# flashlight/wav2letter

Measured on NVIDIA H100. Metric: frames_per_sec, higher is better.
Workload: dtype f32

## Files before the change

### include/w2l_b200.h

```cpp
#ifndef W2L_B200_H_
#define W2L_B200_H_

#include <stddef.h>
#include <stdint.h>

#ifdef __cplusplus
extern "C" {
#endif

#define W2L_API __attribute__((visibility("default")))

enum {
  W2L_OK = 0,
  W2L_ERR_INVALID_ARGUMENT = 1,
  W2L_ERR_WORKSPACE = 2,
  W2L_ERR_CUDA = 3,
  W2L_ERR_UNSUPPORTED = 4
};

enum {
  W2L_SCALE_NONE = 0,
  W2L_SCALE_INPUT_SZ = 1,
  W2L_SCALE_INPUT_SZ_SQRT = 2,
  W2L_SCALE_TARGET_SZ = 3,
// ... 84 lines not shown
W2L_API int w2l_seq2seq_beam_finish(void* stream, int B, int K, int maxlen, int steps, int pad, const void* ws, size_t ws_bytes, int32_t* tokens,
                                    int32_t* lengths, float* scores, int32_t* counts);

W2L_API int w2l_soft_label_loss(void* stream, long long rows, int N, const float* student, const float* teacher, float scale, float* loss_out,
                                float* d_student, float* ws);
W2L_API int w2l_ema_update(void* stream, long long n, float* ema, const float* params, double decay);

W2L_API int w2l_gemm_tf32_view(void* stream, int a_mn_major, int b_mn_major, int M, int N, int K, const float* A, int lda,
                               const float* B, int ldb, float* C, int ldc, const float* bias, int act, int accumulate);
enum { W2L_GEMM_TF32 = 0, W2L_GEMM_F32X3 = 1, W2L_GEMM_BF16 = 2, W2L_GEMM_F32X3_SPLIT_B = 3, W2L_GEMM_FP16 = 4 };
enum { W2L_PRECISION_TF32 = 0, W2L_PRECISION_F32 = 1, W2L_PRECISION_BF16 = 2, W2L_PRECISION_FP16 = 3 };
W2L_API int w2l_set_precision(int precision);
W2L_API int w2l_get_precision(void);
W2L_API int w2l_gemm(void* stream, int kind, int a_mn_major, int b_mn_major, int M, int N, int K, const void* A, int lda,
                     const void* B, int ldb, void* C, int ldc, int c_bf16, const float* bias, int act, int accumulate,
                     const void* aux, int ld_aux, int aux_bf16, int aux_mode, float aux_scale, float dropout_p,
                     unsigned long long seed, int allow_overlap);
W2L_API int w2l_cast_bf16(void* stream, long long n, const float* x, void* y);
W2L_API int w2l_cast_bf16_rows(void* stream, long long rows, int cols, int ld_in, int cols_padded, const float* x, void* y);
W2L_API int w2l_cast_fp16(void* stream, long long n, const float* x, void* y);
W2L_API int w2l_cast_fp16_rows(void* stream, long long rows, int cols, int ld_in, int cols_padded, const float* x, void* y);
W2L_API int w2l_split_tf32(void* stream, int transpose, int rows, int cols, int ld, int cols_padded, const float* x, float* planes);
W2L_API int w2l_gemm_set_tile(int bn);
W2L_API int w2l_gemm_set_variant(int variant);
W2L_API int w2l_gemm_tf32(void* stream, int a_mn_major, int b_mn_major, int M, int N, int K, const float* A, int lda,
                          const float* B, int ldb, float* C, int ldc, const float* bias, int act);

W2L_API int w2l_gemm_tf32_ex(void* stream, int a_mn_major, int b_mn_major, int M, int N, int K, const float* A, int lda,
                             const float* B, int ldb, float* C, int ldc, const float* bias, int act, int accumulate,
                             const float* aux, int ld_aux, int aux_mode, float aux_scale, float dropout_p,
                             unsigned long long seed);

W2L_API size_t w2l_conv_time_workspace_size(int B, int Tout, int Cin, int Cout, int K);
W2L_API int w2l_conv_time_fwd(void* stream, int B, int T, int Tout, int W, int Cin, int Cout, int K, int stride,
                              int pad_left, const float* x, const float* wt, const float* bias, const float* add, float* y,
                              int act, float dropout_p, unsigned long long seed, void* ws, size_t ws_bytes);
W2L_API int w2l_conv_time_dgrad(void* stream, int B, int T, int Tout, int W, int Cin, int Cout, int K, int stride,
                                int pad_left, const float* dy, const float* wt, const float* add, float* dx, void* ws,
                                size_t ws_bytes);
W2L_API int w2l_conv_time_wgrad(void* stream, int B, int T, int Tout, int W, int Cin, int Cout, int K, int stride,
                                int pad_left, const float* x, const float* dy, float* dwt, float* dbias, void* ws,
                                size_t ws_bytes);

W2L_API int w2l_weightnorm_fwd(void* stream, int rows, int len, const float* v, const float* g, float* w, float* inv_norm);
W2L_API int w2l_weightnorm_bwd(void* stream, int rows, int len, const float* v, const float* g, const float* inv_norm,
                               const float* dw, float* dv, float* dg);
// ... 143 lines not shown
```

### wav2letter_b200/capi.py

```python
from __future__ import annotations

import ctypes
import os

import torch

_HERE = os.path.dirname(os.path.abspath(__file__))
LIB_PATH = os.path.join(_HERE, "libw2l_b200.so")

SCALE_MODES = {"none": 0, "input_sz": 1, "input_sz_sqrt": 2, "target_sz": 3, "target_sz_sqrt": 4}
TERM_FCC, TERM_FAC, TERM_ASG = 1, 2, 3

EXPORTS = [
    "w2l_version", "w2l_last_error", "w2l_launch_count", "w2l_reset_launch_count", "w2l_set_profile_events", "w2l_set_profile_event_list", "w2l_profile_events_used", "w2l_trace_begin", "w2l_trace_end", "w2l_trace_list",
    "w2l_asg_workspace_size", "w2l_asg_forward_backward",
    "w2l_asg64_workspace_size", "w2l_asg64_forward_backward",
    "w2l_fcc_viterbi_workspace_size", "w2l_fcc_viterbi",
    "w2l_fcc_viterbi64_workspace_size", "w2l_fcc_viterbi64",
    "w2l_fac_viterbi_workspace_size", "w2l_fac_viterbi",
    "w2l_ctc_workspace_size", "w2l_ctc_forward_backward", "w2l_argmax_path", "w2l_linseg_target",
    "w2l_ctc_viterbi_workspace_size", "w2l_ctc_viterbi_target",
    "w2l_set_precision", "w2l_get_precision", "w2l_gemm", "w2l_cast_bf16", "w2l_cast_bf16_rows", "w2l_cast_fp16", "w2l_cast_fp16_rows", "w2l_split_tf32", "w2l_sgd_step_ex", "w2l_finite_guard",
    "w2l_mask_bands", "w2l_trainer_set_precision", "w2l_trainer_set_grad_stream", "w2l_trainer_set_grad_stream_delay", "w2l_delay", "w2l_trainer_status", "w2l_trainer_save", "w2l_trainer_load", "w2l_trainer_export_streaming",
    "w2l_trainer_set_schedule", "w2l_trainer_set_position", "w2l_trainer_position", "w2l_trainer_set_lr", "w2l_trainer_lr",
    "w2l_trainer_set_amp", "w2l_trainer_amp_state",
    "w2l_text_create", "w2l_text_destroy", "w2l_text_num_classes", "w2l_text_encode", "w2l_text_prediction2ltr", "w2l_text_target2ltr",
    "w2l_text_ltr2wrd", "w2l_text_align_words", "w2l_edit_distance",
    "w2l_gemm_set_variant", "w2l_gemm_set_tile", "w2l_gemm_tf32", "w2l_gemm_tf32_ex", "w2l_gemm_tf32_view", "w2l_conv_time_workspace_size", "w2l_conv_time_fwd", "w2l_conv_time_dgrad",
    "w2l_conv_time_wgrad", "w2l_layernorm_fwd", "w2l_layernorm_rows_fwd", "w2l_layernorm_bwd", "w2l_colsum_accumulate", "w2l_sq_norm_accumulate",
    "w2l_sgd_step", "w2l_weightnorm_fwd", "w2l_weightnorm_bwd", "w2l_conv1d_arrange", "w2l_conv1d_arrange_ex", "w2l_conv1d_unarrange_grad",
    "w2l_glu_fwd", "w2l_glu_bwd", "w2l_prelu_fwd", "w2l_prelu_bwd", "w2l_transpose_input", "w2l_axpy", "w2l_fill", "w2l_act_fwd", "w2l_mask_mul",
    "w2l_trainer_create", "w2l_trainer_destroy", "w2l_trainer_step", "w2l_trainer_forward", "w2l_trainer_num_params",
    "w2l_trainer_param_layout", "w2l_trainer_get_flat", "w2l_trainer_set_flat", "w2l_trainer_sync_parameters",
    "w2l_trainer_describe", "w2l_nccl_unique_id", "w2l_init_distributed", "w2l_trainer_align", "w2l_trainer_time_stride",
    "w2l_mfsc_num_frames", "w2l_mfsc_workspace_size", "w2l_mfsc",
    "w2l_stream_create", "w2l_stream_destroy", "w2l_stream_state_bytes", "w2l_stream_max_frames_out", "w2l_stream_start",
    "w2l_stream_run", "w2l_stream_plan",
    "w2l_mfsc_stream_create", "w2l_mfsc_stream_destroy", "w2l_mfsc_stream_state_bytes", "w2l_mfsc_stream_max_frames_out",
    "w2l_mfsc_stream_start", "w2l_mfsc_stream_run",
    "w2l_seq2seq_check", "w2l_seq2seq_embed_fwd", "w2l_seq2seq_embed_bwd", "w2l_seq2seq_gru_stash_floats", "w2l_seq2seq_gru_fwd",
    "w2l_seq2seq_gru_bwd", "w2l_seq2seq_attn_fwd", "w2l_seq2seq_attn_bwd", "w2l_seq2seq_loss", "w2l_seq2seq_scale_rows",
    "w2l_seq2seq_decode_init", "w2l_seq2seq_decode_step",
    "w2l_seq2seq_beam_workspace_size", "w2l_seq2seq_beam_init", "w2l_seq2seq_beam_step", "w2l_seq2seq_beam_finish",
    "w2l_trainer_create_seq2seq", "w2l_trainer_output_width", "w2l_trainer_seq2seq_config", "w2l_trainer_clear_window",
    "w2l_trainer_seq2seq_seed", "w2l_trainer_decode", "w2l_trainer_beam_search",
    "w2l_seq2seq_sizes", "w2l_seq2seq_attn_fwd_sized", "w2l_seq2seq_attn_bwd_sized", "w2l_trainer_step_sized", "w2l_trainer_decode_sized",
    "w2l_trainer_beam_search_sized",
    "w2l_soft_label_loss", "w2l_ema_update", "w2l_trainer_set_ema", "w2l_trainer_ema", "w2l_trainer_forward_teacher",
    "w2l_trainer_viterbi_path", "w2l_trainer_step_soft",
]

# ... 465 lines not shown
    _check(lib.w2l_cast_fp16_rows(_stream(), x.shape[0], x.shape[1], x.stride(0), cols_padded, _ptr(x), _ptr(y)))
    return y


def split_tf32(x, transpose=False, cols_padded=None):
    if x.dtype != torch.float32 or not x.is_cuda or x.dim() != 2 or x.stride(1) != 1:
        raise TypeError("split_tf32: x must be a 2-D CUDA float32 tensor with contiguous rows")
    rows, cols = x.shape
    k = rows if transpose else cols
    cols_padded = (k + 3) // 4 * 4 if cols_padded is None else cols_padded
    y = torch.empty((2, cols if transpose else rows, cols_padded), dtype=torch.float32, device=x.device)
    _check(lib.w2l_split_tf32(_stream(), int(transpose), rows, cols, x.stride(0), cols_padded, _ptr(x), _ptr(y)))
    return y


def gemm_set_variant(v: int = 1):
    _check(lib.w2l_gemm_set_variant(int(v)))


def gemm_set_tile(bn: int = 0):
    _check(lib.w2l_gemm_set_tile(int(bn)))


def trace(fn, capacity: int = 4096) -> dict:
    _check(lib.w2l_trace_begin(_stream(), capacity))
    try:
        fn()
    finally:
        buf = ctypes.create_string_buffer(1 << 16)
        lib.w2l_trace_end(buf, len(buf))
    out = {}
    for line in buf.value.decode().splitlines():
        name, n, ms = line.split("\t")
        out[name] = (int(n), float(ms))
    return out


def gemm_tf32(A, B, bias=None, act=0, a_mn=False, b_mn=False, out=None):
    A = _req(A, torch.float32, "A")
    B = _req(B, torch.float32, "B")
    bias = _req(bias, torch.float32, "bias")
    M, K = (A.shape[1], A.shape[0]) if a_mn else A.shape
    N = B.shape[1] if b_mn else B.shape[0]
    if out is None:
        out = torch.empty((M, N), dtype=torch.float32, device=A.device)
    _check(lib.w2l_gemm_tf32(_stream(), int(a_mn), int(b_mn), M, N, K, _ptr(A), A.stride(0), _ptr(B), B.stride(0),
# ... 106 lines not shown
```

### wav2letter_b200/csrc/gemm_wgmma.cu

```cuda
#include <cuda.h>
#include <cuda_bf16.h>
#include <cuda_fp16.h>
#include <cuda_runtime.h>

#include <algorithm>
#include <cmath>
#include <cstdlib>
#include <mutex>
#include <type_traits>

#include "common.cuh"
#include "tma_ptx.cuh"
#include "wgmma_ptx.cuh"

namespace w2l {
namespace {
using namespace tma;

constexpr int BM = 128;
constexpr int kRowBytes = 128;
constexpr int kTileBytes = BM * kRowBytes;
constexpr int kGemmThreads = 384;
constexpr int kConvThreads = 96;
constexpr int kConsumerThreads = 256;
enum { kTf32 = W2L_GEMM_TF32, kF32x3 = W2L_GEMM_F32X3, kBf16 = W2L_GEMM_BF16, kF32x3SplitB = W2L_GEMM_F32X3_SPLIT_B, kFp16 = W2L_GEMM_FP16 };
__host__ __device__ constexpr bool k16(int mode) { return mode == kBf16 || mode == kFp16; }
template <int kMode>
using Half = typename std::conditional<kMode == kFp16, __half, __nv_bfloat16>::type;
__device__ __forceinline__ float to_float(__nv_bfloat16 x) { return __bfloat162float(x); }
__device__ __forceinline__ float to_float(__half x) { return __half2float(x); }
template <typename H>
__device__ __forceinline__ H from_float(float x);
template <>
__device__ __forceinline__ __nv_bfloat16 from_float<__nv_bfloat16>(float x) { return __float2bfloat16_rn(x); }
template <>
__device__ __forceinline__ __half from_float<__half>(float x) { return __float2half_rn(x); }
__device__ __forceinline__ void from_float2(float x, float y, __nv_bfloat162* d) { *d = __floats2bfloat162_rn(x, y); }
__device__ __forceinline__ void from_float2(float x, float y, __half2* d) { *d = __floats2half2_rn(x, y); }
template <typename H>
using Half2 = typename std::conditional<std::is_same<H, __half>::value, __half2, __nv_bfloat162>::type;

__host__ __device__ constexpr bool converts(int mode, bool a_mn, bool b_mn) { return mode == kF32x3 || (mode == kTf32 && (a_mn || b_mn)); }
__host__ __device__ constexpr bool a_in_regs(int mode, bool a_mn, bool b_mn) { return converts(mode, a_mn, b_mn) || mode == kF32x3SplitB; }
__host__ __device__ constexpr size_t raw_bytes(int mode, int bn) { return (size_t)kTileBytes + (size_t)bn * kRowBytes * (mode == kF32x3SplitB ? 2 : 1); }
__host__ __device__ constexpr size_t cvt_bytes(int mode, int bn) { return (size_t)bn * kRowBytes * (mode == kF32x3 ? 2 : 1); }
constexpr size_t kSmemTail = 1024 + 256;
constexpr size_t kSmemBudget = 227 * 1024 - kSmemTail;
constexpr int kConvRawStages = 4;
constexpr int kIdSlots = 4;
__host__ __device__ constexpr int raw_stages(int mode, bool a_mn, bool b_mn, int bn) {
  return converts(mode, a_mn, b_mn) ? kConvRawStages
                                    : (kSmemBudget / raw_bytes(mode, bn) > 6 ? 6 : (int)(kSmemBudget / raw_bytes(mode, bn)));
}
__host__ __device__ constexpr int cvt_stages(int mode, bool a_mn, bool b_mn, int bn) {
  return !converts(mode, a_mn, b_mn) ? 0
         : (kSmemBudget - kConvRawStages * raw_bytes(mode, bn)) / cvt_bytes(mode, bn) > 4
             ? 4
             : (int)((kSmemBudget - kConvRawStages * raw_bytes(mode, bn)) / cvt_bytes(mode, bn));
}
__host__ __device__ constexpr size_t smem_for(int mode, bool a_mn, bool b_mn, int bn) {
  return raw_stages(mode, a_mn, b_mn, bn) * raw_bytes(mode, bn) + cvt_stages(mode, a_mn, b_mn, bn) * cvt_bytes(mode, bn) + kSmemTail;
}

struct GemmParams {
  int M, N, K, ldc, act;
  void* C;
  const float* bias;
  int accumulate, aux_mode, ld_aux;
  const void* aux;
  float aux_scale, drop_p;
  unsigned long long seed;
  int k_splits;
  int c_bf16, aux_bf16;
  float* ws;
};

__device__ __forceinline__ uint32_t rn_tf32(uint32_t x) { return (x + 0x1000u) & 0xffffe000u; }

template <bool kMn, bool kLo, int ROWS>
__device__ __forceinline__ void convert_tile(const unsigned char* raw, unsigned char* hi, unsigned char* lo, int ct) {
#pragma unroll 4
  for (int i = ct; i < ROWS * 8; i += kConvThreads) {
    const int r = i % ROWS, c = i / ROWS;
    const uint32_t off = (uint32_t)r * 128u + ((uint32_t)(c ^ (r & 7)) << 4);
// ... 73 lines not shown
    float* part = p.ws + ((size_t)z * p.M + row) * p.N + col;
    part[0] = x0;
    if (two) part[1] = x1;
    return;
  }
  float* dst = static_cast<float*>(p.C) + ci;
  if (two && vec_c) {
    if (p.accumulate) {
      const float2 c = *reinterpret_cast<const float2*>(dst);
      x0 += c.x;
      x1 += c.y;
    }
    *reinterpret_cast<float2*>(dst) = make_float2(x0, x1);
  } else {
    if (p.accumulate) x0 += dst[0];
    dst[0] = x0;
    if (two) {
      if (p.accumulate) x1 += dst[1];
      dst[1] = x1;
    }
  }
}

template <int kMode, bool kAMn, bool kBMn, int BN>
__global__ void __launch_bounds__(kGemmThreads, 1)
gemm_wgmma_kernel(const __grid_constant__ CUtensorMap map_a, const __grid_constant__ CUtensorMap map_b, GemmParams p, int tiles_m, int tiles_n,
                  unsigned int* sched) {
  extern __shared__ __align__(1024) unsigned char smem_raw[];
  unsigned char* smem = reinterpret_cast<unsigned char*>((reinterpret_cast<uintptr_t>(smem_raw) + 1023) & ~(uintptr_t)1023);
  constexpr bool kIs16 = k16(kMode), kPreSplit = kMode == kF32x3SplitB, kSplit = kMode == kF32x3 || kPreSplit;
  constexpr bool kConv = converts(kMode, kAMn, kBMn), kRegA = a_in_regs(kMode, kAMn, kBMn);
  constexpr int BKE = kRowBytes / (kIs16 ? 2 : 4);
  constexpr int kStages = raw_stages(kMode, kAMn, kBMn, BN), kCvtStages = cvt_stages(kMode, kAMn, kBMn, BN);
  constexpr size_t kRaw = raw_bytes(kMode, BN), kCvt = cvt_bytes(kMode, BN);
  constexpr uint32_t kOperandBytes = (uint32_t)kRaw;
  static_assert(kStages >= 2 && (!kConv || kCvtStages >= 2), "gemm: at least two stages per ring");
  static_assert(!kRegA || BN == 128, "gemm: the kinds that take A from registers run at BN = 128");
  static_assert(!kPreSplit || !kBMn, "gemm: pre-split B planes are K-major");
  static_assert(!kIs16 || !kBMn || BN % 64 == 0, "gemm: MN-major 16-bit B is staged in boxes of 64 columns");
  unsigned char* cvt_ring = smem + kStages * kRaw;
  uint64_t* bars = reinterpret_cast<uint64_t*>(cvt_ring + kCvtStages * kCvt);
  uint64_t* full = bars;
  uint64_t* empty = bars + kStages;
  uint64_t* ready = bars + 2 * kStages;
  uint64_t* cvt_empty = ready + kCvtStages;
  uint64_t* id_full = cvt_empty + kCvtStages;
  uint64_t* id_empty = id_full + kIdSlots;
  int* id_ring = reinterpret_cast<int*>(id_empty + kIdSlots);
  static_assert((2 * (kStages + kCvtStages + kIdSlots)) * 8 + kIdSlots * 4 <= kSmemTail - 1024, "gemm: barrier space");
  constexpr uint32_t kIdReaders = kConsumerThreads + (kConv ? kConvThreads : 0);

  const int tid = threadIdx.x, warp = tid >> 5, lane = tid & 31, wg = warp >> 2;
  const int total_kb = (p.K + BKE - 1) / BKE;
  const int kb_per = (total_kb + p.k_splits - 1) / p.k_splits;
  const int tiles_mn = tiles_m * tiles_n, total_tiles = tiles_mn * p.k_splits;

  if (tid == 0) {
    for (int s = 0; s < kStages; ++s) {
// ... 16 lines not shown
  auto next_item = [&]() {
    const int s = id_it % kIdSlots;
    mbar_wait(&id_full[s], (id_it / kIdSlots) & 1);
    const int t = id_ring[s];
    mbar_arrive(&id_empty[s]);
    ++id_it;
    return t;
  };
  auto tile_coords = [&](int t, int& m0, int& n0, int& kb_begin, int& num_kb) {
    const int z = t / tiles_mn, r = t - z * tiles_mn;
    m0 = (r / tiles_n) * BM;
    n0 = (r % tiles_n) * BN;
    kb_begin = z * kb_per;
    int total = total_kb;
    if constexpr (kPreSplit) {
      int k = p.K;
      asm volatile("" : "+r"(k));
      total = (k + BKE - 1) / BKE;
    }
    num_kb = max(0, min(total, kb_begin + kb_per) - kb_begin);
  };

  if (wg == 0) {
    if (warp == 0) {
      if (lane == 0) {
        asm volatile("prefetch.tensormap [%0];" ::"l"(&map_a) : "memory");
        asm volatile("prefetch.tensormap [%0];" ::"l"(&map_b) : "memory");
        uint32_t it = 0;
        for (int t = blockIdx.x; t < total_tiles;) {
          int m0, n0, kb_begin, num_kb;
          tile_coords(t, m0, n0, kb_begin, num_kb);
          for (int kb = 0; kb < num_kb; ++kb, ++it) {
            const int s = it % kStages;
            mbar_wait(&empty[s], ((it / kStages) & 1) ^ 1);
            mbar_expect_tx(&full[s], kOperandBytes);
            unsigned char* sa = smem + s * kRaw;
            unsigned char* sb = sa + kTileBytes;
            const int k0 = (kb_begin + kb) * BKE;
            if (!kAMn) {
              tma_load_2d(&map_a, &full[s], sa, k0, m0);
            } else if (kIs16) {
#pragma unroll
              for (int j = 0; j < BM / 64; ++j) tma_load_2d(&map_a, &full[s], sa + j * 8192, m0 + 64 * j, k0);
            } else {
#pragma unroll
              for (int j = 0; j < BM / 8; ++j) tma_load_2d(&map_a, &full[s], sa + j * 1024, m0 + 8 * j, k0);
// ... 24 lines not shown
            atomicExch(sched + 1, 0u);
          }
        }
      }
    } else if constexpr (kConv) {
      const int ct = tid - 32;
      uint32_t it = 0;
      for (int t = blockIdx.x; t < total_tiles; t = next_item()) {
        int m0, n0, kb_begin, num_kb;
        tile_coords(t, m0, n0, kb_begin, num_kb);
        for (int kb = 0; kb < num_kb; ++kb, ++it) {
          const int s = it % kStages, c = it % kCvtStages;
          mbar_wait(&cvt_empty[c], ((it / kCvtStages) & 1) ^ 1);
          mbar_wait(&full[s], (it / kStages) & 1);
          unsigned char* dst = cvt_ring + c * kCvt;
          convert_tile<kBMn, kSplit, BN>(smem + s * kRaw + kTileBytes, dst, dst + BN * kRowBytes, ct);
          mbar_arrive(&empty[s]);
          asm volatile("fence.proxy.async.shared::cta;" ::: "memory");
          mbar_arrive(&ready[c]);
        }
      }
    }
  } else {
    const int cw = wg - 1;
    const bool vec_c = (p.ldc % 2) == 0 && (reinterpret_cast<uintptr_t>(p.C) & (p.c_bf16 ? 3 : 7)) == 0;
    const int fr = 64 * cw + 16 * (warp & 3) + (lane >> 2), fq = lane & 3;
    uint32_t it = 0;
    for (int t = blockIdx.x; t < total_tiles; t = next_item()) {
      int m0, n0, kb_begin, num_kb;
      tile_coords(t, m0, n0, kb_begin, num_kb);
      float acc[BN / 2];
#pragma unroll
      for (int i = 0; i < BN / 2; ++i) acc[i] = 0.f;
      if constexpr (kRegA) {
        struct AFrag {
          uint32_t hi[4][4], lo[4][4];
        };
        auto fence_frag = [&](AFrag& f) {
          wg::fence_operands(f.hi);
          if constexpr (kSplit) wg::fence_operands(f.lo);
        };
        auto release_b = [&](uint32_t i) {
          if constexpr (kConv) mbar_arrive(&cvt_empty[i % kCvtStages]);
          else mbar_arrive(&empty[i % kStages]);
        };
        auto step = [&](AFrag& cur, AFrag& prev, int kb) {
// ... 18 lines not shown
            mbar_arrive(&empty[s]);
            mbar_wait(&ready[c], (it / kCvtStages) & 1);
            b_base = smem_u32(cvt_ring + c * kCvt);
          } else {
            b_base = sa + kTileBytes;
          }
          fence_frag(cur);
          wg::fence_operands(acc);
          wg::fence();
#pragma unroll
          for (int kk = 0; kk < 4; ++kk) {
            const int sc = (kb | kk) != 0;
            const uint64_t db = make_desc_sw128(b_base + kk * 32, 16, 1024);
            if constexpr (kSplit) {
              wg::mma_tf32_rs<BN>(acc, cur.lo[kk], db, sc);
              wg::mma_tf32_rs<BN>(acc, cur.hi[kk], make_desc_sw128(b_base + BN * kRowBytes + kk * 32, 16, 1024), 1);
              wg::mma_tf32_rs<BN>(acc, cur.hi[kk], db, 1);
            } else {
              wg::mma_tf32_rs<BN>(acc, cur.hi[kk], db, sc);
            }
          }
          wg::commit();
          wg::fence_operands(acc);
          if constexpr (kSplit) wg::wait<1>(); else wg::wait<0>();
          fence_frag(prev);
          if (kb > 0) release_b(it - 1);
          ++it;
        };
        AFrag fa, fb;
        for (int kb = 0; kb < num_kb; kb += 2) {
          step(fa, fb, kb);
          if (kb + 1 < num_kb) step(fb, fa, kb + 1);
        }
        wg::wait<0>();
        wg::fence_operands(acc);
        fence_frag(fa);
        fence_frag(fb);
        if (num_kb > 0) release_b(it - 1);
      } else {
        for (int kb = 0; kb < num_kb; ++kb, ++it) {
          const int s = it % kStages;
          mbar_wait(&full[s], (it / kStages) & 1);
          const uint32_t a_base = smem_u32(smem + s * kRaw) + (uint32_t)(cw * 8192), b_base = smem_u32(smem + s * kRaw) + kTileBytes;
          wg::fence_operands(acc);
          wg::fence();
#pragma unroll
          for (int k = 0; k < 4; ++k) {
            const int sc = (kb | k) != 0;
            if constexpr (kIs16) {
              const uint64_t da = kAMn ? make_desc_sw128(a_base + k * 2048, 8192, 1024) : make_desc_sw128(a_base + k * 32, 16, 1024);
              const uint64_t db = kBMn ? make_desc_sw128(b_base + k * 2048, 8192, 1024) : make_desc_sw128(b_base + k * 32, 16, 1024);
              if constexpr (kMode == kFp16) wg::mma_f16<BN, kAMn ? 1 : 0, kBMn ? 1 : 0>(acc, da, db, sc);
              else wg::mma_bf16<BN, kAMn ? 1 : 0, kBMn ? 1 : 0>(acc, da, db, sc);
            } else {
              wg::mma_tf32<BN>(acc, make_desc_sw128(a_base + k * 32, 16, 1024), make_desc_sw128(b_base + k * 32, 16, 1024), sc);
            }
          }
          wg::commit();
          wg::fence_operands(acc);
          wg::wait<1>();
          if (kb > 0) mbar_arrive(&empty[(it - 1) % kStages]);
// ... 36 lines not shown
                                                         float* __restrict__ y) {
  __shared__ float tile[32][33];
  const int tx = threadIdx.x & 31, ty = threadIdx.x >> 5;
  const int r0 = blockIdx.x * 32, c0 = blockIdx.y * 32;
  if (kT) {
    for (int i = ty; i < 32; i += 8) {
      const int sr = c0 + i, sc = r0 + tx;
      tile[i][tx] = (sr < rows && sc < cols) ? x[(size_t)sr * ld + sc] : 0.f;
    }
    __syncthreads();
  }
  const size_t plane = (size_t)R * ld_out;
  for (int i = ty; i < 32; i += 8) {
    const int r = r0 + i, c = c0 + tx;
    if (r >= R || c >= ld_out) continue;
    const float v = kT ? tile[tx][i] : (c < cols ? x[(size_t)r * ld + c] : 0.f);
    const uint32_t h = rn_tf32(__float_as_uint(v));
    const uint32_t l = rn_tf32(__float_as_uint(v - __uint_as_float(h)));
    y[(size_t)r * ld_out + c] = __uint_as_float(h);
    y[plane + (size_t)r * ld_out + c] = __uint_as_float(l);
  }
}

int make_map(CUtensorMap* map, int mode, bool raw, const void* ptr, long long rows, long long cols, long long ld, int box_cols, int box_rows,
             bool swizzle, int planes = 1) {
  EncodeTiledFn fn = encode_fn();
  if (!fn) return fail(W2L_ERR_CUDA, "gemm: cuTensorMapEncodeTiled entry point not found");
  const int es = k16(mode) ? 2 : 4;
  cuuint64_t dims[3] = {(cuuint64_t)cols, (cuuint64_t)rows, (cuuint64_t)planes};
  cuuint64_t strides[2] = {(cuuint64_t)ld * es, (cuuint64_t)(rows * ld * es)};
  cuuint32_t box[3] = {(cuuint32_t)box_cols, (cuuint32_t)box_rows, 1};
  cuuint32_t estr[3] = {1, 1, 1};
  const CUtensorMapDataType dt = mode == kBf16   ? CU_TENSOR_MAP_DATA_TYPE_BFLOAT16
                                 : mode == kFp16 ? CU_TENSOR_MAP_DATA_TYPE_FLOAT16
                                 : raw           ? CU_TENSOR_MAP_DATA_TYPE_FLOAT32
                                                 : CU_TENSOR_MAP_DATA_TYPE_TFLOAT32;
  CUresult r = fn(map, dt, planes > 1 ? 3 : 2, const_cast<void*>(ptr), dims, strides, box, estr, CU_TENSOR_MAP_INTERLEAVE_NONE,
                  swizzle ? CU_TENSOR_MAP_SWIZZLE_128B : CU_TENSOR_MAP_SWIZZLE_NONE, CU_TENSOR_MAP_L2_PROMOTION_L2_256B,
                  CU_TENSOR_MAP_FLOAT_OOB_FILL_NONE);
  if (r != CUDA_SUCCESS) return fail(W2L_ERR_CUDA, "gemm: cuTensorMapEncodeTiled failed with code " + std::to_string((int)r));
  return W2L_OK;
}

const char* kernel_name(int mode) {
  switch (mode) {
    case kBf16: return "gemm_wgmma_kernel<bf16>";
// ... 7 lines not shown
thread_local int g_variant = 1;

constexpr int kSchedSlots = 64;
__device__ unsigned int g_sched[kSchedSlots][2];
unsigned int* sched_slot(cudaStream_t stream) {
  static std::mutex mu;
  static cudaStream_t owner[kSchedSlots];
  static int used = 0;
  int slot = -1;
  {
    std::lock_guard<std::mutex> lock(mu);
    for (int i = 0; i < used && slot < 0; ++i)
      if (owner[i] == stream) slot = i;
    if (slot < 0 && used < kSchedSlots) {
      owner[used] = stream;
      slot = used++;
    }
  }
  void* base = nullptr;
  if (slot < 0 || cudaGetSymbolAddress(&base, g_sched) != cudaSuccess) return nullptr;
  return static_cast<unsigned int*>(base) + 2 * slot;
}

template <int kMode, bool kAMn, bool kBMn, int BN>
int launch_bn(cudaStream_t stream, const CUtensorMap& ma, const CUtensorMap& mb, const GemmParams& p) {
  constexpr size_t smem = smem_for(kMode, kAMn, kBMn, BN);
  static_assert(smem <= 227 * 1024, "gemm: shared-memory budget");
  static bool configured = false;
  if (!configured) {
    W2L_CUDA_CHECK(cudaFuncSetAttribute(gemm_wgmma_kernel<kMode, kAMn, kBMn, BN>, cudaFuncAttributeMaxDynamicSharedMemorySize, (int)smem));
    configured = true;
  }
  const int tiles_m = (p.M + BM - 1) / BM, tiles_n = (p.N + BN - 1) / BN;
  const int total = tiles_m * tiles_n * p.k_splits;
  const int grid = g_variant == 1 ? std::min(total, sm_count()) : total;
  unsigned int* sched = g_variant == 1 && grid < total ? sched_slot(stream) : nullptr;
  profile_kind(1);
  profile_start(stream);
  gemm_wgmma_kernel<kMode, kAMn, kBMn, BN><<<grid, kGemmThreads, smem, stream>>>(ma, mb, p, tiles_m, tiles_n, sched);
  profile_stop(stream);
  W2L_LAUNCH_CHECK(kernel_name(kMode));
  return W2L_OK;
}
template <int kMode, bool kAMn, bool kBMn>
int launch_mode(cudaStream_t stream, int bn, const CUtensorMap& ma, const CUtensorMap& mb, const GemmParams& p) {
  if constexpr (a_in_regs(kMode, kAMn, kBMn)) {
    return launch_bn<kMode, kAMn, kBMn, 128>(stream, ma, mb, p);
  } else if constexpr (k16(kMode)) {
    return bn <= 128 ? launch_bn<kMode, kAMn, kBMn, 128>(stream, ma, mb, p) : launch_bn<kMode, kAMn, kBMn, 256>(stream, ma, mb, p);
  } else {
    switch (bn) {
      case 128: return launch_bn<kMode, kAMn, kBMn, 128>(stream, ma, mb, p);
      case 160: return launch_bn<kMode, kAMn, kBMn, 160>(stream, ma, mb, p);
      case 224: return launch_bn<kMode, kAMn, kBMn, 224>(stream, ma, mb, p);
      default: return launch_bn<kMode, kAMn, kBMn, 256>(stream, ma, mb, p);
    }
  }
}
template <int kMode>
int launch(cudaStream_t stream, bool a_mn, bool b_mn, int bn, const CUtensorMap& ma, const CUtensorMap& mb, const GemmParams& p) {
  if constexpr (kMode == kF32x3SplitB) {
    return a_mn ? launch_mode<kMode, true, false>(stream, bn, ma, mb, p) : launch_mode<kMode, false, false>(stream, bn, ma, mb, p);
  } else {
    if (!a_mn && !b_mn) return launch_mode<kMode, false, false>(stream, bn, ma, mb, p);
    if (!a_mn && b_mn) return launch_mode<kMode, false, true>(stream, bn, ma, mb, p);
    if (a_mn && b_mn) return launch_mode<kMode, true, true>(stream, bn, ma, mb, p);
    return launch_mode<kMode, true, false>(stream, bn, ma, mb, p);
  }
}

int splits_for(int tiles, int total_kb, bool plain) {
  const int sms = sm_count();
  if (!plain || tiles >= sms || total_kb < 16) return 1;
  return std::max(1, std::min(std::min(sms / tiles, total_kb / 4), 32));
}
thread_local int g_force_bn = 0;
int choose_bn(int mode, bool a_mn, bool b_mn, int M, int N, int total_kb, bool plain, int* splits_out) {
  auto allowed = [&](int bn) {
    if (a_in_regs(mode, a_mn, b_mn)) return bn == 128;
    if (k16(mode)) return bn == 128 || bn == 256;
    return true;
  };
  if (g_force_bn && allowed(g_force_bn)) {
    const int tiles = ((N + g_force_bn - 1) / g_force_bn) * ((M + BM - 1) / BM);
    *splits_out = splits_for(tiles, total_kb, plain);
    return g_force_bn;
  }
  const int cands[4] = {128, 160, 224, 256};
  const double sms = sm_count();
  double best = 1e300;
  int best_bn = 128;
  *splits_out = 1;
  for (int bn : cands) {
    if (!allowed(bn)) continue;
    const int tiles = ((N + bn - 1) / bn) * ((M + BM - 1) / BM);
    const int splits = splits_for(tiles, total_kb, plain);
    const int kb_local = (total_kb + splits - 1) / splits;
    const double waves = std::ceil((double)tiles * splits / sms);
    const double cost = waves * ((double)(128 + bn) * kb_local + 2.0 * bn);
    if (cost < best - 1e-9) {
      best = cost;
      best_bn = bn;
      *splits_out = splits;
    }
  }
  return best_bn;
}

int gemm_impl(void* stream_, int mode, int a_mn_major, int b_mn_major, int M, int N, int K, const void* A, int lda, const void* B, int ldb,
              void* C, int ldc, int c_bf16, const float* bias, int act, int accumulate, const void* aux, int ld_aux, int aux_bf16,
              int aux_mode, float aux_scale, float dropout_p, unsigned long long seed, bool allow_overlap, bool allow_split_k = true) {
  cudaStream_t stream = static_cast<cudaStream_t>(stream_);
  if (mode != kTf32 && mode != kF32x3 && mode != kBf16 && mode != kF32x3SplitB && mode != kFp16) return fail(W2L_ERR_INVALID_ARGUMENT, "gemm: unknown operand kind");
  if (mode == kF32x3SplitB && b_mn_major) return fail(W2L_ERR_INVALID_ARGUMENT, "gemm: F32X3_SPLIT_B takes K-major B planes");
  if (M <= 0 || N <= 0 || K <= 0) return fail(W2L_ERR_INVALID_ARGUMENT, "gemm: M, N, K must be positive");
  if (!A || !B || !C) return fail(W2L_ERR_INVALID_ARGUMENT, "gemm: null pointer");
  if (act < 0 || act > 1) return fail(W2L_ERR_INVALID_ARGUMENT, "gemm: act must be 0 (none) or 1 (relu)");
  if (aux_mode < 0 || aux_mode > 2 || (aux_mode != 0 && (!aux || ld_aux < N)))
    return fail(W2L_ERR_INVALID_ARGUMENT, "gemm: bad aux mask arguments");
  if (dropout_p < 0.f || dropout_p >= 1.f) return fail(W2L_ERR_INVALID_ARGUMENT, "gemm: dropout_p must be in [0, 1)");
  if (dropout_p > 0.f && N % 4 != 0) return fail(W2L_ERR_INVALID_ARGUMENT, "gemm: dropout needs N % 4 == 0");
  const int row_align = k16(mode) ? 8 : 4;
  if ((lda % row_align) || (ldb % row_align) || (reinterpret_cast<uintptr_t>(A) & 15) || (reinterpret_cast<uintptr_t>(B) & 15))
    return fail(W2L_ERR_INVALID_ARGUMENT, "gemm: operand rows must be 16-byte aligned (ld % 4 == 0 for fp32, ld % 8 == 0 for bf16 / fp16)");
  if (ldc < N || (!allow_overlap && (lda < (a_mn_major ? M : K) || ldb < (b_mn_major ? N : K))))
    return fail(W2L_ERR_INVALID_ARGUMENT, "gemm: leading dimension smaller than the row length");
  if (lda <= 0 || ldb <= 0) return fail(W2L_ERR_INVALID_ARGUMENT, "gemm: non-positive leading dimension");
  if (c_bf16 && accumulate) return fail(W2L_ERR_INVALID_ARGUMENT, "gemm: accumulation needs an fp32 C");
  const int bke = kRowBytes / (k16(mode) ? 2 : 4);
  const int total_kb = (K + bke - 1) / bke;
  const bool plain = act == 0 && aux_mode == 0 && dropout_p == 0.f && bias == nullptr && !c_bf16;
  int splits = 1;
  const int BN = choose_bn(mode, a_mn_major != 0, b_mn_major != 0, M, N, total_kb, plain && allow_split_k, &splits);
  const bool raw = a_in_regs(mode, a_mn_major != 0, b_mn_major != 0);
  const bool half = k16(mode);
  CUtensorMap ma, mb;
  int rc;
  if (!a_mn_major)
    rc = make_map(&ma, mode, raw, A, M, K, lda, bke, BM, true);
  else
    rc = make_map(&ma, mode, raw, A, K, M, lda, half ? 64 : 8, bke, half);
  if (rc) return rc;
  if (!b_mn_major)
    rc = make_map(&mb, mode, raw, B, N, K, ldb, bke, BN, true, mode == kF32x3SplitB ? 2 : 1);
  else
    rc = make_map(&mb, mode, raw, B, K, N, ldb, half ? 64 : BN, bke, half);
  if (rc) return rc;
  GemmParams p{M, N, K, ldc, act, C, bias, accumulate, aux_mode, ld_aux, aux, aux_scale, dropout_p, seed, splits, c_bf16, aux_bf16, nullptr};
  if (splits > 1) W2L_CUDA_CHECK(cudaMallocAsync(reinterpret_cast<void**>(&p.ws), sizeof(float) * (size_t)splits * M * N, stream));
  switch (mode) {
    case kBf16: rc = launch<kBf16>(stream, a_mn_major, b_mn_major, BN, ma, mb, p); break;
    case kFp16: rc = launch<kFp16>(stream, a_mn_major, b_mn_major, BN, ma, mb, p); break;
    case kF32x3: rc = launch<kF32x3>(stream, a_mn_major, b_mn_major, BN, ma, mb, p); break;
    case kF32x3SplitB: rc = launch<kF32x3SplitB>(stream, a_mn_major, b_mn_major, BN, ma, mb, p); break;
    default: rc = launch<kTf32>(stream, a_mn_major, b_mn_major, BN, ma, mb, p);
  }
  if (splits > 1) {
    if (rc == W2L_OK) {
      const long long mn = (long long)M * N;
      splitk_reduce_kernel<<<(unsigned)std::min<long long>((mn + 255) / 256, (long long)sm_count() * 8), 256, 0, stream>>>(M, N, splits, p.ws,
                                                                                                                        static_cast<float*>(C), ldc, accumulate);
      cudaError_t e = cudaGetLastError();
      if (e != cudaSuccess) rc = fail(W2L_ERR_CUDA, std::string("launch splitk_reduce_kernel: ") + cudaGetErrorString(e));
      else {
        count_launch();
        trace_launch("splitk_reduce_kernel");
      }
    }
    cudaFreeAsync(p.ws, stream);
  }
  return rc;
}

int f32_kind() { return current_precision() == W2L_PRECISION_F32 ? kF32x3 : kTf32; }

template <typename H>
__global__ void __launch_bounds__(256) cast_kernel(long long n4, const float4* __restrict__ x, uint2* __restrict__ y, long long n,
                                                   const float* __restrict__ xs, H* __restrict__ ys) {
// ... 40 lines not shown
  const unsigned grid = (unsigned)std::min<long long>((total + 255) / 256, (long long)sm_count() * 16);
  cast_rows_kernel<H><<<grid, 256, 0, stream>>>(rows, cols, ld_in, cols_padded, x, static_cast<H*>(y));
  W2L_LAUNCH_CHECK(kname);
  return W2L_OK;
}

}
}

using namespace w2l;

extern "C" int w2l_gemm_set_variant(int variant) {
  if (variant < 0 || variant > 1) return fail(W2L_ERR_INVALID_ARGUMENT, "gemm: variant must be 0 (one tile per CTA) or 1 (one CTA per SM)");
  g_variant = variant;
  return W2L_OK;
}

extern "C" int w2l_gemm_set_tile(int bn) {
  if (bn != 0 && bn != 128 && bn != 160 && bn != 224 && bn != 256) return fail(W2L_ERR_INVALID_ARGUMENT, "gemm: tile width must be 0 (auto), 128, 160, 224 or 256");
  g_force_bn = bn;
  return W2L_OK;
}

extern "C" int w2l_gemm(void* stream, int kind, int a_mn_major, int b_mn_major, int M, int N, int K, const void* A, int lda, const void* B,
                        int ldb, void* C, int ldc, int c_bf16, const float* bias, int act, int accumulate, const void* aux, int ld_aux,
                        int aux_bf16, int aux_mode, float aux_scale, float dropout_p, unsigned long long seed, int allow_overlap) {
  return gemm_impl(stream, kind, a_mn_major, b_mn_major, M, N, K, A, lda, B, ldb, C, ldc, c_bf16, bias, act, accumulate, aux, ld_aux, aux_bf16,
                   aux_mode, aux_scale, dropout_p, seed, allow_overlap != 0);
}

int w2l::gemm_view_unsplit(cudaStream_t stream, int kind, int M, int N, int K, const float* A, int lda, const float* B, int ldb, float* C,
                           int ldc) {
  return gemm_impl(stream, kind, 0, 0, M, N, K, A, lda, B, ldb, C, ldc, 0, nullptr, 0, 0, nullptr, 0, 0, 0, 1.f, 0.f, 0ull, true, false);
}

extern "C" int w2l_gemm_tf32_ex(void* stream_, int a_mn_major, int b_mn_major, int M, int N, int K, const float* A, int lda,
                                const float* B, int ldb, float* C, int ldc, const float* bias, int act, int accumulate,
                                const float* aux, int ld_aux, int aux_mode, float aux_scale, float dropout_p,
                                unsigned long long seed) {
  return gemm_impl(stream_, f32_kind(), a_mn_major, b_mn_major, M, N, K, A, lda, B, ldb, C, ldc, 0, bias, act, accumulate, aux, ld_aux, 0, aux_mode,
                   aux_scale, dropout_p, seed, false);
}

extern "C" int w2l_gemm_tf32(void* stream_, int a_mn_major, int b_mn_major, int M, int N, int K, const float* A, int lda,
                             const float* B, int ldb, float* C, int ldc, const float* bias, int act) {
  return w2l_gemm_tf32_ex(stream_, a_mn_major, b_mn_major, M, N, K, A, lda, B, ldb, C, ldc, bias, act, 0, nullptr, 0, 0, 1.f, 0.f, 0ull);
// ... 1 lines not shown

extern "C" int w2l_gemm_tf32_view(void* stream_, int a_mn_major, int b_mn_major, int M, int N, int K, const float* A, int lda,
                                  const float* B, int ldb, float* C, int ldc, const float* bias, int act, int accumulate) {
  return gemm_impl(stream_, f32_kind(), a_mn_major, b_mn_major, M, N, K, A, lda, B, ldb, C, ldc, 0, bias, act, accumulate, nullptr, 0, 0, 0, 1.f, 0.f,
                   0ull, true);
}

extern "C" int w2l_cast_bf16(void* stream_, long long n, const float* x, void* y) { return cast<__nv_bfloat16>(stream_, n, x, y, "cast_bf16", "cast_bf16_kernel"); }
extern "C" int w2l_cast_bf16_rows(void* stream_, long long rows, int cols, int ld_in, int cols_padded, const float* x, void* y) {
  return cast_rows<__nv_bfloat16>(stream_, rows, cols, ld_in, cols_padded, x, y, "cast_bf16_rows", "cast_bf16_rows_kernel");
}
extern "C" int w2l_cast_fp16(void* stream_, long long n, const float* x, void* y) { return cast<__half>(stream_, n, x, y, "cast_fp16", "cast_fp16_kernel"); }
extern "C" int w2l_cast_fp16_rows(void* stream_, long long rows, int cols, int ld_in, int cols_padded, const float* x, void* y) {
  return cast_rows<__half>(stream_, rows, cols, ld_in, cols_padded, x, y, "cast_fp16_rows", "cast_fp16_rows_kernel");
}
extern "C" int w2l_split_tf32(void* stream_, int transpose, int rows, int cols, int ld, int cols_padded, const float* x, float* planes) {
  if (rows <= 0 || cols <= 0) return W2L_OK;
  if (!x || !planes || ld < cols) return fail(W2L_ERR_INVALID_ARGUMENT, "split_tf32: bad arguments");
  const int R = transpose ? cols : rows;
  if (cols_padded < (transpose ? rows : cols) || (cols_padded + 31) / 32 > 65535)
    return fail(W2L_ERR_INVALID_ARGUMENT, "split_tf32: bad plane size");
  cudaStream_t stream = static_cast<cudaStream_t>(stream_);
  const dim3 grid((unsigned)((R + 31) / 32), (unsigned)((cols_padded + 31) / 32));
  if (transpose)
    split_tf32_kernel<true><<<grid, 256, 0, stream>>>(rows, cols, ld, R, cols_padded, x, planes);
  else
    split_tf32_kernel<false><<<grid, 256, 0, stream>>>(rows, cols, ld, R, cols_padded, x, planes);
  W2L_LAUNCH_CHECK("split_tf32_kernel");
  return W2L_OK;
}
```

Measured before the change: 1.029 million.

## Add 192-row GEMM tiles for split-B F32x3 and vectorized row split kernel

Adds a BM=192 tile variant for the F32X3_SPLIT_B GEMM with three consumer warpgroups. It uses setmaxnreg to move registers from the producer warpgroup to the consumers, and a simpler single-fragment wait loop. A heuristic picks 192-row tiles when doing so reduces wave count enough, to improve operand reuse and wave quantization. It also adds a float4-vectorized non-transposed split_tf32 kernel. The 192-row path drops the overlap between fragment loads and MMA, and the larger smem tiles leave room for fewer pipeline stages.

Result: faster. 1.045 million (median of 6 runs) (+1.5%).

```diff
diff --git a/include/w2l_b200.h b/include/w2l_b200.h
--- a/include/w2l_b200.h
+++ b/include/w2l_b200.h
@@ -130,6 +130,7 @@
 W2L_API int w2l_cast_fp16_rows(void* stream, long long rows, int cols, int ld_in, int cols_padded, const float* x, void* y);
 W2L_API int w2l_split_tf32(void* stream, int transpose, int rows, int cols, int ld, int cols_padded, const float* x, float* planes);
 W2L_API int w2l_gemm_set_tile(int bn);
+W2L_API int w2l_gemm_set_tile_rows(int bm);
 W2L_API int w2l_gemm_set_variant(int variant);
 W2L_API int w2l_gemm_tf32(void* stream, int a_mn_major, int b_mn_major, int M, int N, int K, const float* A, int lda,
                           const float* B, int ldb, float* C, int ldc, const float* bias, int act);
diff --git a/wav2letter_b200/capi.py b/wav2letter_b200/capi.py
--- a/wav2letter_b200/capi.py
+++ b/wav2letter_b200/capi.py
@@ -26,7 +26,7 @@
     "w2l_trainer_set_amp", "w2l_trainer_amp_state",
     "w2l_text_create", "w2l_text_destroy", "w2l_text_num_classes", "w2l_text_encode", "w2l_text_prediction2ltr", "w2l_text_target2ltr",
     "w2l_text_ltr2wrd", "w2l_text_align_words", "w2l_edit_distance",
-    "w2l_gemm_set_variant", "w2l_gemm_set_tile", "w2l_gemm_tf32", "w2l_gemm_tf32_ex", "w2l_gemm_tf32_view", "w2l_conv_time_workspace_size", "w2l_conv_time_fwd", "w2l_conv_time_dgrad",
+    "w2l_gemm_set_variant", "w2l_gemm_set_tile", "w2l_gemm_set_tile_rows", "w2l_gemm_tf32", "w2l_gemm_tf32_ex", "w2l_gemm_tf32_view", "w2l_conv_time_workspace_size", "w2l_conv_time_fwd", "w2l_conv_time_dgrad",
     "w2l_conv_time_wgrad", "w2l_layernorm_fwd", "w2l_layernorm_rows_fwd", "w2l_layernorm_bwd", "w2l_colsum_accumulate", "w2l_sq_norm_accumulate",
     "w2l_sgd_step", "w2l_weightnorm_fwd", "w2l_weightnorm_bwd", "w2l_conv1d_arrange", "w2l_conv1d_arrange_ex", "w2l_conv1d_unarrange_grad",
     "w2l_glu_fwd", "w2l_glu_bwd", "w2l_prelu_fwd", "w2l_prelu_bwd", "w2l_transpose_input", "w2l_axpy", "w2l_fill", "w2l_act_fwd", "w2l_mask_mul",
@@ -538,6 +538,10 @@
     _check(lib.w2l_gemm_set_tile(int(bn)))
 
 
+def gemm_set_tile_rows(bm: int = 0):
+    _check(lib.w2l_gemm_set_tile_rows(int(bm)))
+
+
 def trace(fn, capacity: int = 4096) -> dict:
     _check(lib.w2l_trace_begin(_stream(), capacity))
     try:
diff --git a/wav2letter_b200/csrc/gemm_wgmma.cu b/wav2letter_b200/csrc/gemm_wgmma.cu
--- a/wav2letter_b200/csrc/gemm_wgmma.cu
+++ b/wav2letter_b200/csrc/gemm_wgmma.cu
@@ -17,12 +17,9 @@
 namespace {
 using namespace tma;
 
-constexpr int BM = 128;
 constexpr int kRowBytes = 128;
-constexpr int kTileBytes = BM * kRowBytes;
-constexpr int kGemmThreads = 384;
 constexpr int kConvThreads = 96;
-constexpr int kConsumerThreads = 256;
+__host__ __device__ constexpr int gemm_threads(int bm) { return 2 * bm + 128; }
 enum { kTf32 = W2L_GEMM_TF32, kF32x3 = W2L_GEMM_F32X3, kBf16 = W2L_GEMM_BF16, kF32x3SplitB = W2L_GEMM_F32X3_SPLIT_B, kFp16 = W2L_GEMM_FP16 };
 __host__ __device__ constexpr bool k16(int mode) { return mode == kBf16 || mode == kFp16; }
 template <int kMode>
@@ -42,15 +39,15 @@
 
 __host__ __device__ constexpr bool converts(int mode, bool a_mn, bool b_mn) { return mode == kF32x3 || (mode == kTf32 && (a_mn || b_mn)); }
 __host__ __device__ constexpr bool a_in_regs(int mode, bool a_mn, bool b_mn) { return converts(mode, a_mn, b_mn) || mode == kF32x3SplitB; }
-__host__ __device__ constexpr size_t raw_bytes(int mode, int bn) { return (size_t)kTileBytes + (size_t)bn * kRowBytes * (mode == kF32x3SplitB ? 2 : 1); }
+__host__ __device__ constexpr size_t raw_bytes(int mode, int bn, int bm = 128) { return (size_t)bm * kRowBytes + (size_t)bn * kRowBytes * (mode == kF32x3SplitB ? 2 : 1); }
 __host__ __device__ constexpr size_t cvt_bytes(int mode, int bn) { return (size_t)bn * kRowBytes * (mode == kF32x3 ? 2 : 1); }
 constexpr size_t kSmemTail = 1024 + 256;
 constexpr size_t kSmemBudget = 227 * 1024 - kSmemTail;
 constexpr int kConvRawStages = 4;
 constexpr int kIdSlots = 4;
-__host__ __device__ constexpr int raw_stages(int mode, bool a_mn, bool b_mn, int bn) {
+__host__ __device__ constexpr int raw_stages(int mode, bool a_mn, bool b_mn, int bn, int bm) {
   return converts(mode, a_mn, b_mn) ? kConvRawStages
-                                    : (kSmemBudget / raw_bytes(mode, bn) > 6 ? 6 : (int)(kSmemBudget / raw_bytes(mode, bn)));
+                                    : (kSmemBudget / raw_bytes(mode, bn, bm) > 6 ? 6 : (int)(kSmemBudget / raw_bytes(mode, bn, bm)));
 }
 __host__ __device__ constexpr int cvt_stages(int mode, bool a_mn, bool b_mn, int bn) {
   return !converts(mode, a_mn, b_mn) ? 0
@@ -58,8 +55,8 @@
              ? 4
              : (int)((kSmemBudget - kConvRawStages * raw_bytes(mode, bn)) / cvt_bytes(mode, bn));
 }
-__host__ __device__ constexpr size_t smem_for(int mode, bool a_mn, bool b_mn, int bn) {
-  return raw_stages(mode, a_mn, b_mn, bn) * raw_bytes(mode, bn) + cvt_stages(mode, a_mn, b_mn, bn) * cvt_bytes(mode, bn) + kSmemTail;
+__host__ __device__ constexpr size_t smem_for(int mode, bool a_mn, bool b_mn, int bn, int bm) {
+  return raw_stages(mode, a_mn, b_mn, bn, bm) * raw_bytes(mode, bn, bm) + cvt_stages(mode, a_mn, b_mn, bn) * cvt_bytes(mode, bn) + kSmemTail;
 }
 
 struct GemmParams {
@@ -179,8 +176,8 @@
   }
 }
 
-template <int kMode, bool kAMn, bool kBMn, int BN>
-__global__ void __launch_bounds__(kGemmThreads, 1)
+template <int kMode, bool kAMn, bool kBMn, int BN, int BM>
+__global__ void __launch_bounds__(gemm_threads(BM), 1)
 gemm_wgmma_kernel(const __grid_constant__ CUtensorMap map_a, const __grid_constant__ CUtensorMap map_b, GemmParams p, int tiles_m, int tiles_n,
                   unsigned int* sched) {
   extern __shared__ __align__(1024) unsigned char smem_raw[];
@@ -188,9 +185,13 @@
   constexpr bool kIs16 = k16(kMode), kPreSplit = kMode == kF32x3SplitB, kSplit = kMode == kF32x3 || kPreSplit;
   constexpr bool kConv = converts(kMode, kAMn, kBMn), kRegA = a_in_regs(kMode, kAMn, kBMn);
   constexpr int BKE = kRowBytes / (kIs16 ? 2 : 4);
-  constexpr int kStages = raw_stages(kMode, kAMn, kBMn, BN), kCvtStages = cvt_stages(kMode, kAMn, kBMn, BN);
-  constexpr size_t kRaw = raw_bytes(kMode, BN), kCvt = cvt_bytes(kMode, BN);
+  constexpr int kStages = raw_stages(kMode, kAMn, kBMn, BN, BM), kCvtStages = cvt_stages(kMode, kAMn, kBMn, BN);
+  constexpr size_t kRaw = raw_bytes(kMode, BN, BM), kCvt = cvt_bytes(kMode, BN);
   constexpr uint32_t kOperandBytes = (uint32_t)kRaw;
+  constexpr int kTileBytes = BM * kRowBytes;
+  constexpr int kConsumerThreads = BM * 2;
+  constexpr bool kTall = BM == 192;
+  static_assert(BM == 128 || (kTall && kPreSplit), "gemm: only F32X3_SPLIT_B runs 192-row tiles");
   static_assert(kStages >= 2 && (!kConv || kCvtStages >= 2), "gemm: at least two stages per ring");
   static_assert(!kRegA || BN == 128, "gemm: the kinds that take A from registers run at BN = 128");
   static_assert(!kPreSplit || !kBMn, "gemm: pre-split B planes are K-major");
@@ -253,6 +254,7 @@
   };
 
   if (wg == 0) {
+    if constexpr (kTall) asm volatile("setmaxnreg.dec.sync.aligned.u32 56;" ::: "memory");
     if (warp == 0) {
       if (lane == 0) {
         asm volatile("prefetch.tensormap [%0];" ::"l"(&map_a) : "memory");
@@ -323,6 +325,7 @@
       }
     }
   } else {
+    if constexpr (kTall) asm volatile("setmaxnreg.inc.sync.aligned.u32 152;" ::: "memory");
     const int cw = wg - 1;
     const bool vec_c = (p.ldc % 2) == 0 && (reinterpret_cast<uintptr_t>(p.C) & (p.c_bf16 ? 3 : 7)) == 0;
     const int fr = 64 * cw + 16 * (warp & 3) + (lane >> 2), fq = lane & 3;
@@ -387,21 +390,32 @@
           }
           wg::commit();
           wg::fence_operands(acc);
-          if constexpr (kSplit) wg::wait<1>(); else wg::wait<0>();
-          fence_frag(prev);
-          if (kb > 0) release_b(it - 1);
+          if constexpr (kTall) {
+            wg::wait<0>();
+            fence_frag(cur);
+            release_b(it);
+          } else {
+            if constexpr (kSplit) wg::wait<1>(); else wg::wait<0>();
+            fence_frag(prev);
+            if (kb > 0) release_b(it - 1);
+          }
           ++it;
         };
-        AFrag fa, fb;
-        for (int kb = 0; kb < num_kb; kb += 2) {
-          step(fa, fb, kb);
-          if (kb + 1 < num_kb) step(fb, fa, kb + 1);
+        if constexpr (kTall) {
+          AFrag fa;
+          for (int kb = 0; kb < num_kb; ++kb) step(fa, fa, kb);
+        } else {
+          AFrag fa, fb;
+          for (int kb = 0; kb < num_kb; kb += 2) {
+            step(fa, fb, kb);
+            if (kb + 1 < num_kb) step(fb, fa, kb + 1);
+          }
+          wg::wait<0>();
+          wg::fence_operands(acc);
+          fence_frag(fa);
+          fence_frag(fb);
+          if (num_kb > 0) release_b(it - 1);
         }
-        wg::wait<0>();
-        wg::fence_operands(acc);
-        fence_frag(fa);
-        fence_frag(fb);
-        if (num_kb > 0) release_b(it - 1);
       } else {
         for (int kb = 0; kb < num_kb; ++kb, ++it) {
           const int s = it % kStages;
@@ -484,6 +498,32 @@
   }
 }
 
+__global__ void __launch_bounds__(256) split_tf32_rows_kernel(int rows, int cols, int ld, int ld_out, const float* __restrict__ x,
+                                                              float* __restrict__ y) {
+  const long long q = ld_out / 4, i = (long long)blockIdx.x * blockDim.x + threadIdx.x;
+  if (i >= (long long)rows * q) return;
+  const long long r = i / q;
+  const int c = 4 * (int)(i - r * q);
+  const float* src = x + r * ld + c;
+  float v[4];
+  if (c + 4 <= cols) {
+    const float4 f = __ldg(reinterpret_cast<const float4*>(src));
+    v[0] = f.x, v[1] = f.y, v[2] = f.z, v[3] = f.w;
+  } else {
+#pragma unroll
+    for (int j = 0; j < 4; ++j) v[j] = c + j < cols ? src[j] : 0.f;
+  }
+  uint32_t h[4], l[4];
+#pragma unroll
+  for (int j = 0; j < 4; ++j) {
+    h[j] = rn_tf32(__float_as_uint(v[j]));
+    l[j] = rn_tf32(__float_as_uint(v[j] - __uint_as_float(h[j])));
+  }
+  const size_t at = (size_t)r * ld_out + c;
+  *reinterpret_cast<uint4*>(y + at) = make_uint4(h[0], h[1], h[2], h[3]);
+  *reinterpret_cast<uint4*>(y + (size_t)rows * ld_out + at) = make_uint4(l[0], l[1], l[2], l[3]);
+}
+
 int make_map(CUtensorMap* map, int mode, bool raw, const void* ptr, long long rows, long long cols, long long ld, int box_cols, int box_rows,
              bool swizzle, int planes = 1) {
   EncodeTiledFn fn = encode_fn();
@@ -537,13 +577,13 @@
   return static_cast<unsigned int*>(base) + 2 * slot;
 }
 
-template <int kMode, bool kAMn, bool kBMn, int BN>
+template <int kMode, bool kAMn, bool kBMn, int BN, int BM = 128>
 int launch_bn(cudaStream_t stream, const CUtensorMap& ma, const CUtensorMap& mb, const GemmParams& p) {
-  constexpr size_t smem = smem_for(kMode, kAMn, kBMn, BN);
+  constexpr size_t smem = smem_for(kMode, kAMn, kBMn, BN, BM);
   static_assert(smem <= 227 * 1024, "gemm: shared-memory budget");
   static bool configured = false;
   if (!configured) {
-    W2L_CUDA_CHECK(cudaFuncSetAttribute(gemm_wgmma_kernel<kMode, kAMn, kBMn, BN>, cudaFuncAttributeMaxDynamicSharedMemorySize, (int)smem));
+    W2L_CUDA_CHECK(cudaFuncSetAttribute(gemm_wgmma_kernel<kMode, kAMn, kBMn, BN, BM>, cudaFuncAttributeMaxDynamicSharedMemorySize, (int)smem));
     configured = true;
   }
   const int tiles_m = (p.M + BM - 1) / BM, tiles_n = (p.N + BN - 1) / BN;
@@ -552,7 +592,7 @@
   unsigned int* sched = g_variant == 1 && grid < total ? sched_slot(stream) : nullptr;
   profile_kind(1);
   profile_start(stream);
-  gemm_wgmma_kernel<kMode, kAMn, kBMn, BN><<<grid, kGemmThreads, smem, stream>>>(ma, mb, p, tiles_m, tiles_n, sched);
+  gemm_wgmma_kernel<kMode, kAMn, kBMn, BN, BM><<<grid, gemm_threads(BM), smem, stream>>>(ma, mb, p, tiles_m, tiles_n, sched);
   profile_stop(stream);
   W2L_LAUNCH_CHECK(kernel_name(kMode));
   return W2L_OK;
@@ -573,8 +613,9 @@
   }
 }
 template <int kMode>
-int launch(cudaStream_t stream, bool a_mn, bool b_mn, int bn, const CUtensorMap& ma, const CUtensorMap& mb, const GemmParams& p) {
+int launch(cudaStream_t stream, bool a_mn, bool b_mn, int bn, int bm, const CUtensorMap& ma, const CUtensorMap& mb, const GemmParams& p) {
   if constexpr (kMode == kF32x3SplitB) {
+    if (bm == 192) return a_mn ? launch_bn<kMode, true, false, 128, 192>(stream, ma, mb, p) : launch_bn<kMode, false, false, 128, 192>(stream, ma, mb, p);
     return a_mn ? launch_mode<kMode, true, false>(stream, bn, ma, mb, p) : launch_mode<kMode, false, false>(stream, bn, ma, mb, p);
   } else {
     if (!a_mn && !b_mn) return launch_mode<kMode, false, false>(stream, bn, ma, mb, p);
@@ -597,7 +638,7 @@
     return true;
   };
   if (g_force_bn && allowed(g_force_bn)) {
-    const int tiles = ((N + g_force_bn - 1) / g_force_bn) * ((M + BM - 1) / BM);
+    const int tiles = ((N + g_force_bn - 1) / g_force_bn) * ((M + 127) / 128);
     *splits_out = splits_for(tiles, total_kb, plain);
     return g_force_bn;
   }
@@ -608,7 +649,7 @@
   *splits_out = 1;
   for (int bn : cands) {
     if (!allowed(bn)) continue;
-    const int tiles = ((N + bn - 1) / bn) * ((M + BM - 1) / BM);
+    const int tiles = ((N + bn - 1) / bn) * ((M + 127) / 128);
     const int splits = splits_for(tiles, total_kb, plain);
     const int kb_local = (total_kb + splits - 1) / splits;
     const double waves = std::ceil((double)tiles * splits / sms);
@@ -620,6 +661,14 @@
     }
   }
   return best_bn;
+}
+constexpr double kTall192 = 1.38;
+thread_local int g_force_bm = 0;
+int choose_bm(int M, int N) {
+  if (g_force_bm) return g_force_bm;
+  const int sms = sm_count(), tiles_n = (N + 127) / 128;
+  const int waves128 = ((M + 127) / 128 * tiles_n + sms - 1) / sms, waves192 = ((M + 191) / 192 * tiles_n + sms - 1) / sms;
+  return waves192 * kTall192 < waves128 ? 192 : 128;
 }
 
 int gemm_impl(void* stream_, int mode, int a_mn_major, int b_mn_major, int M, int N, int K, const void* A, int lda, const void* B, int ldb,
@@ -647,6 +696,7 @@
   const bool plain = act == 0 && aux_mode == 0 && dropout_p == 0.f && bias == nullptr && !c_bf16;
   int splits = 1;
   const int BN = choose_bn(mode, a_mn_major != 0, b_mn_major != 0, M, N, total_kb, plain && allow_split_k, &splits);
+  const int BM = mode == kF32x3SplitB && splits == 1 ? choose_bm(M, N) : 128;
   const bool raw = a_in_regs(mode, a_mn_major != 0, b_mn_major != 0);
   const bool half = k16(mode);
   CUtensorMap ma, mb;
@@ -664,11 +714,11 @@
   GemmParams p{M, N, K, ldc, act, C, bias, accumulate, aux_mode, ld_aux, aux, aux_scale, dropout_p, seed, splits, c_bf16, aux_bf16, nullptr};
   if (splits > 1) W2L_CUDA_CHECK(cudaMallocAsync(reinterpret_cast<void**>(&p.ws), sizeof(float) * (size_t)splits * M * N, stream));
   switch (mode) {
-    case kBf16: rc = launch<kBf16>(stream, a_mn_major, b_mn_major, BN, ma, mb, p); break;
-    case kFp16: rc = launch<kFp16>(stream, a_mn_major, b_mn_major, BN, ma, mb, p); break;
-    case kF32x3: rc = launch<kF32x3>(stream, a_mn_major, b_mn_major, BN, ma, mb, p); break;
-    case kF32x3SplitB: rc = launch<kF32x3SplitB>(stream, a_mn_major, b_mn_major, BN, ma, mb, p); break;
-    default: rc = launch<kTf32>(stream, a_mn_major, b_mn_major, BN, ma, mb, p);
+    case kBf16: rc = launch<kBf16>(stream, a_mn_major, b_mn_major, BN, BM, ma, mb, p); break;
+    case kFp16: rc = launch<kFp16>(stream, a_mn_major, b_mn_major, BN, BM, ma, mb, p); break;
+    case kF32x3: rc = launch<kF32x3>(stream, a_mn_major, b_mn_major, BN, BM, ma, mb, p); break;
+    case kF32x3SplitB: rc = launch<kF32x3SplitB>(stream, a_mn_major, b_mn_major, BN, BM, ma, mb, p); break;
+    default: rc = launch<kTf32>(stream, a_mn_major, b_mn_major, BN, BM, ma, mb, p);
   }
   if (splits > 1) {
     if (rc == W2L_OK) {
@@ -755,6 +805,12 @@
   return W2L_OK;
 }
 
+extern "C" int w2l_gemm_set_tile_rows(int bm) {
+  if (bm != 0 && bm != 128 && bm != 192) return fail(W2L_ERR_INVALID_ARGUMENT, "gemm: tile rows must be 0 (auto), 128 or 192");
+  g_force_bm = bm;
+  return W2L_OK;
+}
+
 extern "C" int w2l_gemm(void* stream, int kind, int a_mn_major, int b_mn_major, int M, int N, int K, const void* A, int lda, const void* B,
                         int ldb, void* C, int ldc, int c_bf16, const float* bias, int act, int accumulate, const void* aux, int ld_aux,
                         int aux_bf16, int aux_mode, float aux_scale, float dropout_p, unsigned long long seed, int allow_overlap) {
@@ -802,8 +858,11 @@
     return fail(W2L_ERR_INVALID_ARGUMENT, "split_tf32: bad plane size");
   cudaStream_t stream = static_cast<cudaStream_t>(stream_);
   const dim3 grid((unsigned)((R + 31) / 32), (unsigned)((cols_padded + 31) / 32));
+  const bool rows16 = ld % 4 == 0 && cols_padded % 4 == 0 && (reinterpret_cast<uintptr_t>(x) & 15) == 0 && (reinterpret_cast<uintptr_t>(planes) & 15) == 0;
   if (transpose)
     split_tf32_kernel<true><<<grid, 256, 0, stream>>>(rows, cols, ld, R, cols_padded, x, planes);
+  else if (rows16)
+    split_tf32_rows_kernel<<<(unsigned)(((long long)rows * (cols_padded / 4) + 255) / 256), 256, 0, stream>>>(rows, cols, ld, cols_padded, x, planes);
   else
     split_tf32_kernel<false><<<grid, 256, 0, stream>>>(rows, cols, ld, R, cols_padded, x, planes);
   W2L_LAUNCH_CHECK("split_tf32_kernel");
```
